# alasdairtran/transform-and-tell

Hardware: AMD Instinct MI355X
Metric: training samples/sec (img+article->caption) (higher is better)
Workload: dtype bf16; 1 GPU; BASELINE configs[2] (= per-GPU shape of configs[3]): expt/nytimes/9_transformer_objects - full faces+objects model (4 contexts: ResNet-152 image regions, RoBERTa-large article with the 25-layer weigh_bert mix, 4 faces, 64 objects), batch 32/GPU, 512-token articles, 32 caption steps; full step = frozen encoders fwd + decoder fwd/loss/bwd + BertAdam; global_batch=32, article_len=512, caption_len=33, parallelism=dp1, step_graph_replays=193, skipped_steps=0

## Files before the change

### transform-and-tell_amd/csrc/attention.hip

```cpp
#include "common.h"
#include "options.h"
#include <type_traits>

template <typename T, int D> struct ACfg {
  static constexpr int VEC = Elem<T>::VEC;
  static constexpr int PAD = sizeof(T) == 2 ? 8 : 1;
  static constexpr int DS = D + PAD;
  static constexpr int SS = 32 + PAD;
  static constexpr int DP = D < 32 ? 32 : D;
  static constexpr int DF = DP / 32;
};

typedef __attribute__((ext_vector_type(2))) float f32x2_t;
typedef __attribute__((ext_vector_type(2))) __bf16 bf16x2_t;
__device__ __forceinline__ unsigned pack_bf16x2(float lo, float hi) {
  f32x2_t f = {lo, hi};
  bf16x2_t h = __builtin_convertvector(f, bf16x2_t);
  return *reinterpret_cast<unsigned*>(&h);
}
template <typename T, int KD>
__device__ __forceinline__ f32x16 mma32(f32x16 acc, const T* a, int as, const T* b, int bs, int lane) {
  if constexpr (sizeof(T) == 2) {
#pragma unroll
    for (int ks = 0; ks < KD; ks += 16) {
// ... 678 lines not shown
            for (int r = 0; r < 16; r += 2) {
              float k0, k1;
              tell_keep2(p.seed, salt_eff, base + (f * 32 + (r & 3) + 8 * (r >> 2)), p.thr, p.inv_keep, k0, k1);
              st[f][r] = k0 != 0.f ? st[f][r] : 0.f;
              st[f][r + 1] = k1 != 0.f ? st[f][r + 1] : 0.f;
            }
        } else {
#pragma unroll
          for (int f = 0; f < 2; ++f)
#pragma unroll
            for (int r = 0; r < 16; ++r)
              st[f][r] = tell_keep(p.seed, salt_eff, base + (f * 32 + (r & 3) + 8 * (r >> 2)), p.thr, p.inv_keep) != 0.f
                             ? st[f][r] : 0.f;
        }
      }
      ls += __shfl_xor(ls, 32, 64);
      l_run = l_run * alpha + ls;
      m_run = m_new;
      if (__any(alpha != 1.f)) {
#pragma unroll
        for (int f = 0; f < 2; ++f)
#pragma unroll
          for (int r = 0; r < 16; ++r) o[f][r] *= alpha;
      }
#pragma unroll
      for (int f = 0; f < 2; ++f)
#pragma unroll
        for (int j = 0; j < 2; ++j) {
          typedef __attribute__((ext_vector_type(4))) unsigned int pk4;
          const pk4 w = {pack_bf16x2(st[f][8 * j], st[f][8 * j + 1]), pack_bf16x2(st[f][8 * j + 2], st[f][8 * j + 3]),
                         pack_bf16x2(st[f][8 * j + 4], st[f][8 * j + 5]), pack_bf16x2(st[f][8 * j + 6], st[f][8 * j + 7])};
          const bf16x8 pf = __builtin_bit_cast(bf16x8, w);
          const T* vrow = Vb + (f * 32 + j * 16) * VS;
#pragma unroll
          for (int dt = 0; dt < 2; ++dt) {
            const bf16x8 vf = attn_tr_frag(vrow + dt * 32, vrow + 8 * VS + dt * 32);
            o[dt] = __builtin_amdgcn_mfma_f32_32x32x16_bf16(vf, pf, o[dt], 0, 0, 0);
          }
        }
    }
    if (kt + 1 < nkt) RSTORE_TILE(kt + 1, buf ^ 1)
    __syncthreads();
  }
#undef RLOAD_TILE
#undef RSTORE_TILE
  if (!active || t >= p.Tq) return;
  const float inv_l = (l_run > 0.f ? 1.f / l_run : 0.f) * (DROP ? p.inv_keep : 1.f);
  T* og = static_cast<T*>(p.out) + t * p.o_st + b * p.o_sb + (long)h * D;
#pragma unroll
  for (int dt = 0; dt < 2; ++dt)
#pragma unroll
    for (int g = 0; g < 4; ++g) {
      const int d0 = dt * 32 + 8 * g + 4 * hh;
      uint2 w;
      w.x = pack_bf16x2(o[dt][4 * g] * inv_l, o[dt][4 * g + 1] * inv_l);
      w.y = pack_bf16x2(o[dt][4 * g + 2] * inv_l, o[dt][4 * g + 3] * inv_l);
      *reinterpret_cast<uint2*>(og + d0) = w;
    }
  if (lane < 32 && p.lse) p.lse[(long)bh * p.Tq + t] = l_run > 0.f ? m_run + __logf(l_run) : INFINITY;
}

#define ATTN_SELF_THR 8.0f
typedef __attribute__((address_space(3))) void* attn_lds_ptr_t;
typedef const __attribute__((address_space(1))) void* attn_glb_ptr_t;
template <bool DROP, int ABL = 0, bool DMA = false>
__global__ __launch_bounds__(256, 3) void attn_self_fwd_kernel(AttnArgs p) {
  const uint32_t salt_eff = tell_step_salt(p.salt, p.step);
  using T = uint16_t;
  constexpr int D = 64, KT = 64, NW = 4;
  constexpr int KS = DMA ? 64 : 72, VS = DMA ? 64 : 96;
  __shared__ __attribute__((aligned(16))) T Ks[2][KT * KS];
  __shared__ __attribute__((aligned(16))) T Vs[2][KT * VS];
  __shared__ __attribute__((aligned(16))) float key_bias[2][KT];
  __shared__ int tile_masked[2];
  typedef __attribute__((ext_vector_type(4))) unsigned int u32x4;
  typedef __attribute__((ext_vector_type(4))) float f32x4;
  typedef __attribute__((ext_vector_type(2))) float f32x2;

  const int tid = threadIdx.x, lane = tid & 63, wave = tid >> 6, hh = lane >> 5, qi = lane & 31;
  const int bh = blockIdx.y, b = bh / p.H, h = bh % p.H;
  const int QB = (p.Tq + 31) / 32;
  const int qb = blockIdx.x * NW + wave;
  const bool active = qb < QB;
  const int t = qb * 32 + qi;
  const int nkt = p.S / KT;
  const T* qg = static_cast<const T*>(p.q);
  const T* kb = static_cast<const T*>(p.k) + (long)b * p.k_sb + (long)h * D;
  const T* vb = static_cast<const T*>(p.v) + (long)b * p.v_sb + (long)h * D;
  const uint8_t* mrow = p.mask ? p.mask + (long)b * p.S : nullptr;

  bf16x8 qf[4];
  {
    const bool ok = active && t < p.Tq;
    const T* qp = ok ? qg + (long)t * p.q_st + (long)b * p.q_sb + (long)h * D : qg;
    const u32x4 zero4 = {0u, 0u, 0u, 0u};
#pragma unroll
    for (int ks = 0; ks < 4; ++ks) {
      u32x4 v = *reinterpret_cast<const u32x4*>(qp + (ok ? 16 * ks + 8 * hh : 0));
      if (!ok) v = zero4;
      qf[ks] = __builtin_bit_cast(bf16x8, v);
    }
  }
  unsigned koff[2], voff[2];
#pragma unroll
  for (int i = 0; i < 2; ++i) {
    const int c = tid + 256 * i;
    if constexpr (DMA) {
      const int row = 8 * (2 * wave + i) + (lane >> 3), ch = (lane & 7) ^ (row & 7);
      koff[i] = (unsigned)(row * (int)p.k_ss + ch * 8);
      voff[i] = (unsigned)(row * (int)p.v_ss + ch * 8);
    } else {
      koff[i] = (unsigned)((c >> 3) * (int)p.k_ss + (c & 7) * 8);
      voff[i] = (unsigned)((c >> 3) * (int)p.v_ss + (c & 7) * 8);
    }
  }
  const int kw0 = (tid >> 3) * KS + (tid & 7) * 8, vw0 = (tid >> 3) * VS + (tid & 7) * 8;
  u32x4 rk[2], rv[2];
  auto rload = [&](int kt) __attribute__((always_inline)) {
    const T* kt_b = kb + (long)kt * KT * p.k_ss;
    const T* vt_b = vb + (long)kt * KT * p.v_ss;
#pragma unroll
    for (int i = 0; i < 2; ++i) {
      rk[i] = *reinterpret_cast<const u32x4*>(kt_b + koff[i]);
      rv[i] = *reinterpret_cast<const u32x4*>(vt_b + voff[i]);
    }
  };
  auto dma = [&](int kt, auto buf_c) __attribute__((always_inline)) {
    constexpr int BUF = decltype(buf_c)::value;
    const T* kt_b = kb + (long)kt * KT * p.k_ss;
    const T* vt_b = vb + (long)kt * KT * p.v_ss;
#pragma unroll
    for (int i = 0; i < 2; ++i) {
      __builtin_amdgcn_global_load_lds((attn_glb_ptr_t)(kt_b + koff[i]), (attn_lds_ptr_t)&Ks[BUF][8 * (2 * wave + i) * KS], 16, 0, 0);
      __builtin_amdgcn_global_load_lds((attn_glb_ptr_t)(vt_b + voff[i]), (attn_lds_ptr_t)&Vs[BUF][8 * (2 * wave + i) * VS], 16, 0, 0);
    }
  };
  auto rstore = [&](int kt, auto buf_c) __attribute__((always_inline)) {
    constexpr int BUF = decltype(buf_c)::value;
    if constexpr (!DMA) {
#pragma unroll
      for (int i = 0; i < 2; ++i) {
        *reinterpret_cast<u32x4*>(&Ks[BUF][kw0 + i * 32 * KS]) = rk[i];
        *reinterpret_cast<u32x4*>(&Vs[BUF][vw0 + i * 32 * VS]) = rv[i];
      }
    } else {
      asm volatile("s_waitcnt vmcnt(0)" ::: "memory");
    }
    if (tid < KT) {
      const bool ok = mrow ? mrow[kt * KT + tid] == 0 : true;
      key_bias[BUF][tid] = ok ? 0.f : -INFINITY;
      const bool any_masked = __ballot(!ok) != 0;
      if (tid == 0) tile_masked[BUF] = any_masked;
    }
  };
  using B0 = std::integral_constant<int, 0>;
  using B1 = std::integral_constant<int, 1>;
  if constexpr (DMA) dma(0, B0{}); else rload(0);
  rstore(0, B0{});
  __syncthreads();

  f32x16 o[2];
#pragma unroll
  for (int f = 0; f < 2; ++f)
#pragma unroll
    for (int r = 0; r < 16; ++r) o[f][r] = 0.f;
  float m_run = -INFINITY, l_run = 0.f;
  const int k_off = qi * KS + 8 * hh;
  const int v_off = (4 * hh + ((lane & 15) >> 2)) * VS + 16 * ((lane >> 4) & 1) + 4 * (lane & 3);
  int k_sw[4], v_sw[2][2];
#pragma unroll
  for (int ks = 0; ks < 4; ++ks) k_sw[ks] = qi * 64 + (((2 * ks + hh) ^ (qi & 7)) << 3);
#pragma unroll
  for (int half = 0; half < 2; ++half)
#pragma unroll
    for (int dt = 0; dt < 2; ++dt) {
      const int r = 8 * half + 4 * hh + ((lane & 15) >> 2), c = dt * 32 + 16 * ((lane >> 4) & 1) + 4 * (lane & 3);
      v_sw[half][dt] = r * 64 + (((c >> 3) ^ (r & 7)) << 3) + (c & 7);
    }
  const uint64_t row_base = ((uint64_t)bh * p.Tq + t) * (uint64_t)p.S + 4 * hh;
  constexpr float LOG2E = 1.4426950408889634f;

  auto tile = [&](int kt, auto buf_c) __attribute__((always_inline)) {
    constexpr int BUF = decltype(buf_c)::value;
    if ((ABL & 2) == 0 && kt + 1 < nkt) {
      if constexpr (DMA) {
        if constexpr (BUF == 0) dma(kt + 1, B1{}); else dma(kt + 1, B0{});
      } else {
        rload(kt + 1);
      }
    }
    if (active) {
      const T* Kb = &Ks[BUF][k_off];
      const T* Vb = &Vs[BUF][v_off];
      f32x16 st[2];
#pragma unroll
      for (int f = 0; f < 2; ++f)
#pragma unroll
        for (int r = 0; r < 16; ++r) st[f][r] = 0.f;
#pragma unroll
      for (int ks = 0; ks < 4; ++ks)
#pragma unroll
        for (int f = 0; f < 2; ++f) {
          const bf16x8 kf = DMA ? *reinterpret_cast<const bf16x8*>(&Ks[BUF][f * 32 * 64 + k_sw[ks]])
                                : *reinterpret_cast<const bf16x8*>(Kb + f * 32 * KS + 16 * ks);
          st[f] = __builtin_amdgcn_mfma_f32_32x32x16_bf16(kf, qf[ks], st[f], 0, 0, 0);
        }
      if (__builtin_amdgcn_readfirstlane(tile_masked[BUF])) {
#pragma unroll
        for (int f = 0; f < 2; ++f)
#pragma unroll
          for (int g = 0; g < 4; ++g) {
            const f32x4 kb4 = *reinterpret_cast<const f32x4*>(&key_bias[BUF][f * 32 + 8 * g + 4 * hh]);
#pragma unroll
            for (int e = 0; e < 4; ++e) st[f][4 * g + e] += kb4[e];
          }
      }
      float mx = fmaxf(st[0][0], st[0][1]);
#pragma unroll
      for (int r = 2; r < 16; r += 2) mx = fmaxf(fmaxf(mx, st[0][r]), st[0][r + 1]);
#pragma unroll
      for (int r = 0; r < 16; r += 2) mx = fmaxf(fmaxf(mx, st[1][r]), st[1][r + 1]);
      mx = fmaxf(mx, __shfl_xor(mx, 32, 64));
      const float m_cand = fmaxf(m_run, mx);
      if (__any(!(m_cand - m_run <= ATTN_SELF_THR))) {
        const float alpha = (m_run == -INFINITY) ? 0.f : __expf(m_run - m_cand);
        m_run = m_cand;
        l_run *= alpha;
#pragma unroll
        for (int f = 0; f < 2; ++f)
#pragma unroll
          for (int r = 0; r < 16; ++r) o[f][r] *= alpha;
      }
      const float neg_m = (m_run == -INFINITY) ? 0.f : -m_run * LOG2E;
      f32x2 ls2 = {0.f, 0.f};
#pragma unroll
      for (int f = 0; f < 2; ++f)
#pragma unroll
        for (int r = 0; r < 16; r += 2) {
          const f32x2 s2 = {st[f][r], st[f][r + 1]};
          const f32x2 e2 = s2 * LOG2E + neg_m;
          const f32x2 pv = {__builtin_amdgcn_exp2f(e2[0]), __builtin_amdgcn_exp2f(e2[1])};
          ls2 += pv;
          st[f][r] = pv[0];
          st[f][r + 1] = pv[1];
        }
      float ls = ls2[0] + ls2[1];
      if constexpr (DROP) {
        const uint64_t base = row_base + (uint64_t)kt * KT;
        if (tell_keep_row_ok(base >> 2, 16)) {
          const TellKeepRow row = tell_keep_row(p.seed, salt_eff, base >> 2);
          uint32_t x = row.x0;
#pragma unroll
          for (int f = 0; f < 2; ++f)
#pragma unroll
            for (int r = 0; r < 16; r += 4) {
              bool k0, k1, k2, k3;
              tell_keep4_bits(x, row.y, p.thr, k0, k1, k2, k3);
              st[f][r] = k0 ? st[f][r] : 0.f;
              st[f][r + 1] = k1 ? st[f][r + 1] : 0.f;
              st[f][r + 2] = k2 ? st[f][r + 2] : 0.f;
              st[f][r + 3] = k3 ? st[f][r + 3] : 0.f;
              x += 2u * TELL_QUAD_STRIDE;
            }
        } else {
#pragma unroll
          for (int f = 0; f < 2; ++f)
#pragma unroll
            for (int r = 0; r < 16; r += 2) {
              float k0, k1;
              tell_keep2(p.seed, salt_eff, base + (f * 32 + (r & 3) + 8 * (r >> 2)), p.thr, p.inv_keep, k0, k1);
              st[f][r] = k0 != 0.f ? st[f][r] : 0.f;
              st[f][r + 1] = k1 != 0.f ? st[f][r + 1] : 0.f;
            }
        }
      }
      ls += __shfl_xor(ls, 32, 64);
      l_run += ls;
#pragma unroll
      for (int f = 0; f < 2; ++f)
#pragma unroll
        for (int j = 0; j < 2; ++j) {
          typedef __attribute__((ext_vector_type(4))) unsigned int pk4;
          const pk4 w = {pack_bf16x2(st[f][8 * j], st[f][8 * j + 1]), pack_bf16x2(st[f][8 * j + 2], st[f][8 * j + 3]),
                         pack_bf16x2(st[f][8 * j + 4], st[f][8 * j + 5]), pack_bf16x2(st[f][8 * j + 6], st[f][8 * j + 7])};
          const bf16x8 pf = __builtin_bit_cast(bf16x8, w);
          const T* vrow = Vb + (f * 32 + j * 16) * VS;
#pragma unroll
          for (int dt = 0; dt < 2; ++dt) {
            const T* vt = &Vs[BUF][(f * 32 + j * 16) * 64];
            const bf16x8 vf = DMA ? attn_tr_frag(vt + v_sw[0][dt], vt + v_sw[1][dt])
                                  : attn_tr_frag(vrow + dt * 32, vrow + 8 * VS + dt * 32);
            o[dt] = __builtin_amdgcn_mfma_f32_32x32x16_bf16(vf, pf, o[dt], 0, 0, 0);
          }
        }
    }
    if ((ABL & 2) == 0 && kt + 1 < nkt) {
      if constexpr (BUF == 0) rstore(kt + 1, B1{}); else rstore(kt + 1, B0{});
    }
    if ((ABL & 1) == 0) __syncthreads();
  };
  for (int kt = 0; kt < nkt; kt += 2) {
    tile(kt, B0{});
    if (kt + 1 < nkt) tile(kt + 1, B1{});
  }
  if (!active || t >= p.Tq) return;
  const float inv_l = (l_run > 0.f ? 1.f / l_run : 0.f) * (DROP ? p.inv_keep : 1.f);
  T* og = static_cast<T*>(p.out) + (long)t * p.o_st + (long)b * p.o_sb + (long)h * D;
#pragma unroll
  for (int dt = 0; dt < 2; ++dt)
#pragma unroll
    for (int g = 0; g < 4; ++g) {
      const int d0 = dt * 32 + 8 * g + 4 * hh;
      uint2 w;
      w.x = pack_bf16x2(o[dt][4 * g] * inv_l, o[dt][4 * g + 1] * inv_l);
      w.y = pack_bf16x2(o[dt][4 * g + 2] * inv_l, o[dt][4 * g + 3] * inv_l);
      *reinterpret_cast<uint2*>(og + d0) = w;
    }
  if (lane < 32 && p.lse) p.lse[(long)bh * p.Tq + t] = l_run > 0.f ? m_run + __logf(l_run) : INFINITY;
}

__device__ __forceinline__ bf16x8 attn_km_frag(const uint16_t* tile, int ld, int m0, int ks, int lane) {
  const uint16_t* p = tile + (ks + 8 * (lane >> 5) + ((lane & 15) >> 2)) * ld + m0 + 16 * ((lane >> 4) & 1) + 4 * (lane & 3);
  return attn_tr_frag(p, p + 4 * ld);
}
__device__ __forceinline__ f32x16 mma32_kmA(f32x16 acc, const uint16_t* a_km, int ald, int m0, const uint16_t* b, int bs, int lane) {
#pragma unroll
  for (int ks = 0; ks < 32; ks += 16) {
    const bf16x8 av = attn_km_frag(a_km, ald, m0, ks, lane);
    const bf16x8 bv = *reinterpret_cast<const bf16x8*>(b + (lane & 31) * bs + ks + ((lane >> 5) << 3));
    acc = __builtin_amdgcn_mfma_f32_32x32x16_bf16(av, bv, acc, 0, 0, 0);
  }
  return acc;
}
__device__ __forceinline__ f32x16 mma32_kmB(f32x16 acc, const uint16_t* a, int as, const uint16_t* b_km, int bld, int n0, int lane) {
#pragma unroll
  for (int ks = 0; ks < 32; ks += 16) {
    const bf16x8 av = *reinterpret_cast<const bf16x8*>(a + (lane & 31) * as + ks + ((lane >> 5) << 3));
    const bf16x8 bv = attn_km_frag(b_km, bld, n0, ks, lane);
    acc = __builtin_amdgcn_mfma_f32_32x32x16_bf16(av, bv, acc, 0, 0, 0);
  }
  return acc;
}

template <typename T, int D, int NW>
__global__ __launch_bounds__(64 * NW, (sizeof(T) == 2 && D == 64 && NW == 4) ? 2 : 1) void attn_bwd_kernel(AttnArgs p) {
  const uint32_t salt_eff = tell_step_salt(p.salt, p.step);
  using C_ = ACfg<T, D>;
  constexpr int DS = C_::DS, SS = C_::SS, DP = C_::DP, DF = C_::DF;
  constexpr bool TR = sizeof(T) == 2 && D == 64;
  constexpr int SHARED_ELEMS = 2 * 32 * DS + (TR ? 0 : 2 * DP * SS);
  constexpr int WAVE_ELEMS = 2 * 32 * DS + (TR ? 0 : DP * SS) + 3 * 32 * SS;
  static_assert(WAVE_ELEMS * sizeof(T) >= 16 * DF * 64 * sizeof(float), "dQ combine buffer must fit");
  __shared__ __attribute__((aligned(16))) T smem[SHARED_ELEMS + NW * WAVE_ELEMS];
  __shared__ float lse_s[32], delta_s[32];
  __shared__ float key_ok[NW][32];

  const int tid = threadIdx.x, lane = tid & 63, wave = tid >> 6;
  const int bh = blockIdx.x, b = bh / p.H, h = bh % p.H;
  const int QB = (p.Tq + 31) / 32;
  const int S_total = p.S + p.has_bias + p.has_zero;
  const int nkt = (S_total + 31) / 32;
  const int iters = (nkt + NW - 1) / NW;
  const int qi = lane & 31;

  T* Qs = smem;
  T* dOs = Qs + 32 * DS;
  T* Qt = dOs + 32 * DS;
  T* dOt = Qt + (TR ? 0 : DP * SS);
  T* Ks = smem + SHARED_ELEMS + wave * WAVE_ELEMS;
  T* Vs = Ks + 32 * DS;
  T* Kt = Vs + 32 * DS;
  T* PdT = Kt + (TR ? 0 : DP * SS);
  T* dST = PdT + 32 * SS;
  T* dSs = dST + 32 * SS;
  const T* qg = static_cast<const T*>(p.q);
  const T* kg = static_cast<const T*>(p.k);
  const T* vg = static_cast<const T*>(p.v);
  const T* og = static_cast<const T*>(p.o);
  const T* dog = static_cast<const T*>(p.dout);
  const T* bk = static_cast<const T*>(p.bias_k);
  const T* bv = static_cast<const T*>(p.bias_v);

  if (DP > D) {
    zero_lds(Qt, 2 * DP * SS, tid, 64 * NW);
    zero_lds(Kt, DP * SS, lane, 64);
  }

  for (int qb = 0; qb < QB; ++qb) {
    const int q0 = qb * 32;
    __syncthreads();
    Tile32Regs<T, D> rk, rv;
    auto fetch = [&](int kt_) __attribute__((always_inline)) {
      const int s0_ = kt_ * 32;
      load32<T, D>(rk, lane, [&](int row) -> const T* {
        int s = s0_ + row;
        if (s < p.S) return kg + s * p.k_ss + b * p.k_sb + (long)h * D;
        if (s == p.S && p.has_bias) return bk + (long)h * D;
        return nullptr;
      }, qg);
      load32<T, D>(rv, lane, [&](int row) -> const T* {
        int s = s0_ + row;
        if (s < p.S) return vg + s * p.v_ss + b * p.v_sb + (long)h * D;
        if (s == p.S && p.has_bias) return bv + (long)h * D;
        return nullptr;
      }, qg);
    };
    if (wave < nkt) fetch(wave);
    {
      constexpr int VEC = Elem<T>::VEC, CPR = D / VEC;
      static_assert((32 * CPR) % 64 == 0 && CPR <= 16 && (CPR & (CPR - 1)) == 0, "whole waves, rows inside a wave");
      for (int c = tid; c < 32 * CPR; c += 64 * NW) {
        const int row = c / CPR, ch = c % CPR, t = q0 + row;
        const bool ok = t < p.Tq;
        const long qo = ok ? t * p.q_st + b * p.q_sb + (long)h * D + ch * VEC : 0;
        const long oo = ok ? t * p.o_st + b * p.o_sb + (long)h * D + ch * VEC : 0;
        uint4 vq = *reinterpret_cast<const uint4*>(qg + qo);
        uint4 vdo = *reinterpret_cast<const uint4*>((ok ? dog : qg) + oo);
        uint4 vo = *reinterpret_cast<const uint4*>((ok ? og : qg) + oo);
        const float lse_row = p.lse[(long)bh * p.Tq + (ok ? t : 0)];
        if (!ok) vq = vdo = vo = make_uint4(0, 0, 0, 0);
        float fdo[VEC], fo[VEC];
        unpack16(vdo, fdo, (const T*)nullptr);
        unpack16(vo, fo, (const T*)nullptr);
        float part = 0.f;
#pragma unroll
        for (int k = 0; k < VEC; ++k) part += fdo[k] * fo[k];
#pragma unroll
        for (int o = CPR / 2; o > 0; o >>= 1) part += __shfl_xor(part, o, 64);
        if (ch == 0) {
          delta_s[row] = part;
          lse_s[row] = ok ? lse_row : INFINITY;
        }
        if constexpr (sizeof(T) == 2) {
          *reinterpret_cast<uint4*>(Qs + row * DS + ch * VEC) = vq;
          *reinterpret_cast<uint4*>(dOs + row * DS + ch * VEC) = vdo;
        } else {
          float* q1 = reinterpret_cast<float*>(Qs) + row * DS + ch * VEC;
          float* q2 = reinterpret_cast<float*>(dOs) + row * DS + ch * VEC;
          q1[0] = __uint_as_float(vq.x); q1[1] = __uint_as_float(vq.y); q1[2] = __uint_as_float(vq.z); q1[3] = __uint_as_float(vq.w);
          q2[0] = __uint_as_float(vdo.x); q2[1] = __uint_as_float(vdo.y); q2[2] = __uint_as_float(vdo.z); q2[3] = __uint_as_float(vdo.w);
        }
        if constexpr (!TR) {
          const T* eq = reinterpret_cast<const T*>(&vq);
          const T* ed = reinterpret_cast<const T*>(&vdo);
#pragma unroll
          for (int k = 0; k < VEC; ++k) {
            Qt[(ch * VEC + k) * SS + row] = eq[k];
            dOt[(ch * VEC + k) * SS + row] = ed[k];
          }
        }
      }
    }
    f32x16 dq[DF];
#pragma unroll
    for (int f = 0; f < DF; ++f)
#pragma unroll
      for (int r = 0; r < 16; ++r) dq[f][r] = 0.f;

    for (int it = 0; it < iters; ++it) {
      const int kt = it * NW + wave;
      const bool tv = kt < nkt;
      const int s0 = kt * 32;
      __syncthreads();
      if (tv) {
        store32<T, D>(rk, Ks, DS, TR ? (T*)nullptr : Kt, SS, lane);
        store32<T, D>(rv, Vs, DS, (T*)nullptr, 0, lane);
        if (kt + NW < nkt) fetch(kt + NW);
        if (lane < 32) {
          const int s = s0 + lane;
          bool ok = s < S_total;
          if (ok && s < p.S && p.mask) ok = p.mask[(long)b * p.S + s] == 0;
          key_ok[wave][lane] = ok ? 1.f : 0.f;
        }
      }
      __syncthreads();
      if (tv) {
        f32x16 st, dp;
#pragma unroll
        for (int r = 0; r < 16; ++r) { st[r] = 0.f; dp[r] = 0.f; }
        st = mma32<T, D>(st, Ks, DS, Qs, DS, lane);
        dp = mma32<T, D>(dp, Vs, DS, dOs, DS, lane);
        const float lse = lse_s[qi], delta = delta_s[qi];
        const int t = q0 + qi;
        float keepv[16], dsv[16];
        if (p.thr) {
          const uint64_t base = ((uint64_t)bh * p.Tq + t) * S_total + s0;
          if ((S_total & 1) == 0) {
#pragma unroll
            for (int r = 0; r < 16; r += 2)
              tell_keep2(p.seed, salt_eff, base + acc_row(r, lane), p.thr, p.inv_keep, keepv[r], keepv[r + 1]);
          } else {
#pragma unroll
            for (int r = 0; r < 16; ++r) keepv[r] = tell_keep(p.seed, salt_eff, base + acc_row(r, lane), p.thr, p.inv_keep);
          }
        } else {
#pragma unroll
          for (int r = 0; r < 16; ++r) keepv[r] = 1.f;
        }
#pragma unroll
        for (int r = 0; r < 16; ++r) {
          const int kk = acc_row(r, lane);
          const bool ok = key_ok[wave][kk] != 0.f && t < p.Tq;
          const float pv = ok ? __expf(st[r] - lse) : 0.f;
          const float keep = keepv[r];
          const float ds = pv * (dp[r] * keep - delta);
          Elem<T>::st(PdT + kk * SS + qi, pv * keep);
          Elem<T>::st(dST + kk * SS + qi, ds);
          dsv[r] = ds;
        }
#pragma unroll
        for (int g = 0; g < 4; ++g) {
          T* pd = dSs + qi * SS + 8 * g + 4 * (lane >> 5);
          if constexpr (sizeof(T) == 2) {
            uint2 w;
            w.x = pack_bf16x2(dsv[4 * g], dsv[4 * g + 1]);
            w.y = pack_bf16x2(dsv[4 * g + 2], dsv[4 * g + 3]);
            *reinterpret_cast<uint2*>(pd) = w;
          } else {
#pragma unroll
            for (int e = 0; e < 4; ++e) Elem<T>::st(pd + e, dsv[4 * g + e]);
          }
        }
      }
      __syncthreads();
      if (tv) {
#pragma unroll
        for (int f = 0; f < DF; ++f) {
          f32x16 dv, dk;
#pragma unroll
          for (int r = 0; r < 16; ++r) { dv[r] = 0.f; dk[r] = 0.f; }
          if constexpr (TR) {
            dv = mma32_kmA(dv, dOs, DS, f * 32, PdT, SS, lane);
            dk = mma32_kmA(dk, Qs, DS, f * 32, dST, SS, lane);
            dq[f] = mma32_kmB(dq[f], dSs, SS, Ks, DS, f * 32, lane);
          } else {
            dv = mma32<T, 32>(dv, dOt + f * 32 * SS, SS, PdT, SS, lane);
            dk = mma32<T, 32>(dk, Qt + f * 32 * SS, SS, dST, SS, lane);
            dq[f] = mma32<T, 32>(dq[f], dSs, SS, Kt + f * 32 * SS, SS, lane);
          }
          const int s = s0 + (lane & 31);
          const bool real = s < p.S, isb = s == p.S && p.has_bias;
          T* pk = static_cast<T*>(p.dk) + (real ? s * p.k_ss + b * p.k_sb : 0) + (long)h * D;
          T* pv_ = static_cast<T*>(p.dv) + (real ? s * p.v_ss + b * p.v_sb : 0) + (long)h * D;
          float* gk = p.dbias_k ? p.dbias_k + (long)b * p.dbias_ld + (long)h * D : nullptr;
          float* gv = p.dbias_v ? p.dbias_v + (long)b * p.dbias_ld + (long)h * D : nullptr;
#pragma unroll
          for (int g = 0; g < 4; ++g) {
            const int d0 = f * 32 + 8 * g + 4 * (lane >> 5);
            if (d0 >= D) continue;
            float vk[4], vv[4];
#pragma unroll
            for (int e = 0; e < 4; ++e) { vk[e] = dk[4 * g + e]; vv[e] = dv[4 * g + e]; }
            if (real) {
              if (qb != 0) {
#pragma unroll
                for (int e = 0; e < 4; ++e) { vk[e] += Elem<T>::ld(pk + d0 + e); vv[e] += Elem<T>::ld(pv_ + d0 + e); }
              }
              if constexpr (sizeof(T) == 2) {
                uint2 wk, wv;
                wk.x = pack_bf16x2(vk[0], vk[1]); wk.y = pack_bf16x2(vk[2], vk[3]);
                wv.x = pack_bf16x2(vv[0], vv[1]); wv.y = pack_bf16x2(vv[2], vv[3]);
                *reinterpret_cast<uint2*>(pk + d0) = wk;
                *reinterpret_cast<uint2*>(pv_ + d0) = wv;
              } else {
                *reinterpret_cast<float4*>(pk + d0) = make_float4(vk[0], vk[1], vk[2], vk[3]);
                *reinterpret_cast<float4*>(pv_ + d0) = make_float4(vv[0], vv[1], vv[2], vv[3]);
              }
            } else if (isb) {
              float4* qk = reinterpret_cast<float4*>(gk + d0);
              float4* qv = reinterpret_cast<float4*>(gv + d0);
              if (qb == 0) {
                *qk = make_float4(vk[0], vk[1], vk[2], vk[3]);
                *qv = make_float4(vv[0], vv[1], vv[2], vv[3]);
              } else {
                const float4 ok_ = *qk, ov_ = *qv;
                *qk = make_float4(ok_.x + vk[0], ok_.y + vk[1], ok_.z + vk[2], ok_.w + vk[3]);
                *qv = make_float4(ov_.x + vv[0], ov_.y + vv[1], ov_.z + vv[2], ov_.w + vv[3]);
              }
            }
          }
        }
      }
    }
    __syncthreads();
    float* comb = reinterpret_cast<float*>(smem + SHARED_ELEMS + wave * WAVE_ELEMS);
#pragma unroll
    for (int f = 0; f < DF; ++f)
#pragma unroll
      for (int r = 0; r < 16; ++r) comb[(f * 16 + r) * 64 + lane] = dq[f][r];
    __syncthreads();
    for (int item = wave; item < DF * 16; item += NW) {
      float s = 0.f;
      for (int w = 0; w < NW; ++w)
        s += reinterpret_cast<const float*>(smem + SHARED_ELEMS + w * WAVE_ELEMS)[item * 64 + lane];
      const int f = item / 16, r = item % 16;
      const int t = q0 + acc_row(r, lane), d = f * 32 + (lane & 31);
      if (t < p.Tq && d < D)
        Elem<T>::st(static_cast<T*>(p.dq) + t * p.q_st + b * p.q_sb + (long)h * D + d, s);
    }
  }
}

template <typename T>
__global__ __launch_bounds__(256) void attn_avg_weights_kernel(const T* __restrict__ q, const T* __restrict__ k,
                                                               const float* __restrict__ lse,
                                                               const uint8_t* __restrict__ mask,
                                                               const T* __restrict__ bias_k,
                                                               float* __restrict__ w, int B, int H, int Tq,
                                                               int S, int D, long q_st, long q_sb, long k_ss,
                                                               long k_sb, int has_bias, int has_zero) {
  const int t = blockIdx.x, b = blockIdx.y;
  const int S_total = S + has_bias + has_zero;
  for (int s = threadIdx.x; s < S_total; s += 256) {
    float acc = 0.f;
    const bool masked = s < S && mask && mask[(long)b * S + s];
    if (!masked) {
      for (int h = 0; h < H; ++h) {
        const T* qp = q + t * q_st + b * q_sb + (long)h * D;
        const T* kp = s < S ? k + s * k_ss + b * k_sb + (long)h * D
                            : (s == S && has_bias ? bias_k + (long)h * D : nullptr);
        float dot = 0.f;
        if (kp) for (int d = 0; d < D; ++d) dot += Elem<T>::ld(qp + d) * Elem<T>::ld(kp + d);
        acc += __expf(dot - lse[((long)b * H + h) * Tq + t]);
      }
    }
    w[((long)b * Tq + t) * S_total + s] = acc / H;
  }
}
extern "C" int tell_attn_avg_weights(const void* q, const void* k, const float* lse, const uint8_t* mask,
                                     const void* bias_k, float* w, int B, int H, int Tq, int S, int D,
                                     long q_st, long q_sb, long k_ss, long k_sb, int has_zero, int dtype,
                                     hipStream_t stream) {
  if (B * Tq <= 0) return TELL_OK;
  dim3 grid(Tq, B);
  if (dtype == TELL_BF16)
    hipLaunchKernelGGL((attn_avg_weights_kernel<uint16_t>), grid, dim3(256), 0, stream, (const uint16_t*)q, (const uint16_t*)k, lse, mask, (const uint16_t*)bias_k, w, B, H, Tq, S, D, q_st, q_sb, k_ss, k_sb, bias_k ? 1 : 0, has_zero);
  else
    hipLaunchKernelGGL((attn_avg_weights_kernel<float>), grid, dim3(256), 0, stream, (const float*)q, (const float*)k, lse, mask, (const float*)bias_k, w, B, H, Tq, S, D, q_st, q_sb, k_ss, k_sb, bias_k ? 1 : 0, has_zero);
  return tell_check_launch("attn_avg_weights");
}

static int fill_args(AttnArgs& a, const void* q, const void* k, const void* v, void* out, float* lse,
                     const uint8_t* mask, const void* bias_k, const void* bias_v, int B, int H, int Tq,
                     int S, int D, long q_st, long q_sb, long k_ss, long k_sb, long v_ss, long v_sb,
                     long o_st, long o_sb, int has_zero, float p, uint32_t seed, uint32_t salt, int dtype) {
  TELL_REQUIRE(D == 64 || D == 16, "attention: head_dim must be 64 (or 16 for the reduced-size tests)");
  TELL_REQUIRE(B > 0 && H > 0 && Tq > 0 && S >= 0, "attention: bad sizes");
  TELL_REQUIRE((bias_k == nullptr) == (bias_v == nullptr), "attention: bias_k and bias_v go together");
  TELL_REQUIRE(S + (bias_k ? 1 : 0) + has_zero > 0, "attention: no keys");
  TELL_REQUIRE(p >= 0.f && p < 1.f, "attention: dropout p must be in [0,1)");
  const int vec = dtype == TELL_BF16 ? 8 : 4;
  TELL_REQUIRE(q_st % vec == 0 && q_sb % vec == 0 && k_ss % vec == 0 && k_sb % vec == 0 &&
               v_ss % vec == 0 && v_sb % vec == 0, "attention: strides must be multiples of a 16-byte chunk");
  TELL_REQUIRE(((uintptr_t)q & 15) == 0 && ((uintptr_t)k & 15) == 0 && ((uintptr_t)v & 15) == 0,
               "attention: q/k/v must be 16-byte aligned");
  a.q = q; a.k = k; a.v = v; a.out = out; a.lse = lse; a.mask = mask; a.bias_k = bias_k; a.bias_v = bias_v;
  a.q_st = q_st; a.q_sb = q_sb; a.k_ss = k_ss; a.k_sb = k_sb; a.v_ss = v_ss; a.v_sb = v_sb;
  a.o_st = o_st; a.o_sb = o_sb; a.B = B; a.H = H; a.Tq = Tq; a.S = S;
  a.has_bias = bias_k ? 1 : 0; a.has_zero = has_zero;
  a.thr = p > 0.f ? tell_drop_threshold(p) : 0u; a.inv_keep = 1.f / (1.f - p); a.seed = seed; a.salt = salt; a.step = g_tell_rng_step;
  a.dout = nullptr; a.o = nullptr; a.dq = a.dk = a.dv = nullptr; a.dbias_k = a.dbias_v = nullptr; a.dbias_ld = 0;
  return TELL_OK;
}

extern "C" int tell_attn_fwd(const void* q, const void* k, const void* v, void* out, float* lse,
                             const uint8_t* mask, const void* bias_k, const void* bias_v, int B, int H,
                             int Tq, int S, int D, long q_st, long q_sb, long k_ss, long k_sb, long v_ss,
                             long v_sb, long o_st, long o_sb, int has_zero, float p, uint32_t seed,
                             uint32_t salt, int dtype, hipStream_t stream) {
  AttnArgs a;
  int rc = fill_args(a, q, k, v, out, lse, mask, bias_k, bias_v, B, H, Tq, S, D, q_st, q_sb, k_ss, k_sb,
                     v_ss, v_sb, o_st, o_sb, has_zero, p, seed, salt, dtype);
  if (rc) return rc;
  const int QB = (Tq + 31) / 32;
  if (D == 64 && QB >= 4) {
    dim3 grid((QB + 3) / 4, B * H);
    const int old_path = (int)tell_opt(OPT_ATTN_TILE64);
    const bool self_env = tell_opt(OPT_ATTN_SELF) != 0;
    if (dtype == TELL_BF16 && !old_path && self_env && !a.has_bias && !a.has_zero && S % 64 == 0 &&
        (long)63 * k_ss + 64 < (1L << 31) && (long)63 * v_ss + 64 < (1L << 31)) {
      const bool dma_env = tell_opt(OPT_ATTN_DMA) == 1;
      if (dma_env) {
        if (a.thr) hipLaunchKernelGGL((attn_self_fwd_kernel<true, 0, true>), grid, dim3(256), 0, stream, a);
        else hipLaunchKernelGGL((attn_self_fwd_kernel<false, 0, true>), grid, dim3(256), 0, stream, a);
      } else if (a.thr) {
        hipLaunchKernelGGL((attn_self_fwd_kernel<true>), grid, dim3(256), 0, stream, a);
      } else hipLaunchKernelGGL((attn_self_fwd_kernel<false>), grid, dim3(256), 0, stream, a);
      return tell_check_launch("attn_self_fwd");
    }
    if (dtype == TELL_BF16 && !old_path) {
      const int occ = (int)tell_opt(OPT_ATTN_OCC);
      if (occ == 3) {
        if (a.thr) hipLaunchKernelGGL((attn_fwd_reg_kernel<true, 3>), grid, dim3(256), 0, stream, a);
        else hipLaunchKernelGGL((attn_fwd_reg_kernel<false, 3>), grid, dim3(256), 0, stream, a);
      } else if (a.thr) hipLaunchKernelGGL((attn_fwd_reg_kernel<true>), grid, dim3(256), 0, stream, a);
      else hipLaunchKernelGGL((attn_fwd_reg_kernel<false>), grid, dim3(256), 0, stream, a);
      return tell_check_launch("attn_fwd_reg");
    } else if (dtype == TELL_BF16) {
      if (a.thr) hipLaunchKernelGGL((attn_fwd_tile64_kernel<uint16_t, true>), grid, dim3(256), 0, stream, a);
      else hipLaunchKernelGGL((attn_fwd_tile64_kernel<uint16_t, false>), grid, dim3(256), 0, stream, a);
    } else {
      if (a.thr) hipLaunchKernelGGL((attn_fwd_tile64_kernel<float, true>), grid, dim3(256), 0, stream, a);
      else hipLaunchKernelGGL((attn_fwd_tile64_kernel<float, false>), grid, dim3(256), 0, stream, a);
    }
    return tell_check_launch("attn_fwd_tile64");
  }
  if (dtype == TELL_BF16) {
    constexpr int NW = 4;
    dim3 grid(QB == 1 ? 1 : (QB + NW - 1) / NW, B * H);
    if (D == 64) hipLaunchKernelGGL((attn_fwd_kernel<uint16_t, 64, NW>), grid, dim3(64 * NW), 0, stream, a);
    else hipLaunchKernelGGL((attn_fwd_kernel<uint16_t, 16, NW>), grid, dim3(64 * NW), 0, stream, a);
  } else {
    constexpr int NW = 4;
    dim3 grid(QB == 1 ? 1 : (QB + NW - 1) / NW, B * H);
    if (D == 64) hipLaunchKernelGGL((attn_fwd_kernel<float, 64, NW>), grid, dim3(64 * NW), 0, stream, a);
    else hipLaunchKernelGGL((attn_fwd_kernel<float, 16, NW>), grid, dim3(64 * NW), 0, stream, a);
  }
  return tell_check_launch("attn_fwd");
}

extern "C" int tell_attn_bwd(const void* q, const void* k, const void* v, const void* out,
                             const void* dout, const float* lse, const uint8_t* mask, const void* bias_k,
                             const void* bias_v, void* dq, void* dk, void* dv, float* dbias_k,
                             float* dbias_v, int B, int H, int Tq, int S, int D, long q_st, long q_sb,
                             long k_ss, long k_sb, long v_ss, long v_sb, long o_st, long o_sb,
                             int has_zero, float p, uint32_t seed, uint32_t salt, int dtype,
                             hipStream_t stream) {
  AttnArgs a;
  int rc = fill_args(a, q, k, v, const_cast<void*>(out), const_cast<float*>(lse), mask, bias_k, bias_v, B,
                     H, Tq, S, D, q_st, q_sb, k_ss, k_sb, v_ss, v_sb, o_st, o_sb, has_zero, p, seed, salt,
                     dtype);
  if (rc) return rc;
  TELL_REQUIRE(!bias_k || (dbias_k && dbias_v), "attention bwd: dbias buffers required with bias rows");
  a.dout = dout; a.o = out; a.dq = dq; a.dk = dk; a.dv = dv; a.dbias_k = dbias_k; a.dbias_v = dbias_v;
  a.dbias_ld = (dbias_k && dbias_v == dbias_k + (long)H * D) ? 2L * H * D : (long)H * D;
  dim3 grid(B * H);
  if (dtype == TELL_BF16) {
    const int nkt = (S + (bias_k ? 1 : 0) + has_zero + 31) / 32;
    if (D == 64 && nkt <= 1) hipLaunchKernelGGL((attn_bwd_kernel<uint16_t, 64, 1>), grid, dim3(64), 0, stream, a);
    else if (D == 64 && nkt <= 4) hipLaunchKernelGGL((attn_bwd_kernel<uint16_t, 64, 2>), grid, dim3(128), 0, stream, a);
    else if (D == 64) hipLaunchKernelGGL((attn_bwd_kernel<uint16_t, 64, 4>), grid, dim3(256), 0, stream, a);
    else hipLaunchKernelGGL((attn_bwd_kernel<uint16_t, 16, 4>), grid, dim3(256), 0, stream, a);
  } else {
    if (D == 64) hipLaunchKernelGGL((attn_bwd_kernel<float, 64, 2>), grid, dim3(128), 0, stream, a);
    else hipLaunchKernelGGL((attn_bwd_kernel<float, 16, 2>), grid, dim3(128), 0, stream, a);
  }
  return tell_check_launch("attn_bwd");
}
```

### transform-and-tell_amd/csrc/options.h

```cpp
#pragma once
#include <atomic>

#define TELL_OPTION_LIST(X)                                                                                             \
                                  \
  X(OPT_GEMM_Q4, "gemm_q4", 1)                               \
  X(OPT_GEMM_Q4E, "gemm_q4e", 1)                         \
  X(OPT_Q4_PARTIAL, "q4_partial", 1)                                                 \
  X(OPT_Q4_DYNAMIC, "q4_dynamic", 0)        \
  X(OPT_Q4_VAR, "q4_var", 0)                \
  X(OPT_GEMM_PP2, "gemm_pp2", 2)                \
  X(OPT_PP2_DYNAMIC, "pp2_dynamic", 1)                                                                                  \
  X(OPT_PP2_GRID, "pp2_grid", 0)                          \
  X(OPT_GEMM_PERSIST, "gemm_persist", 0)                                                                                \
  X(OPT_GEMM_TILE, "gemm_tile", 0)          \
                                                                \
  X(OPT_GEMM_S64, "gemm_s64", 1)                                \
  X(OPT_GEMM_SMALL, "gemm_small", 1)                                                                                    \
  X(OPT_GEMM_RING, "gemm_ring", 0)               \
  X(OPT_GEMM_SPLITK, "gemm_splitk", -1)                                                                                 \
  X(OPT_GROUP_TILE, "group_tile", 0)                                                                                    \
  X(OPT_GROUP_WIDE, "group_wide", 1)                                                                                    \
  X(OPT_GROUP_SORT, "group_sort", 1)                                                                                    \
  X(OPT_CONV_TILE, "conv_tile", 0)                  \
  X(OPT_BN_FUSE, "bn_fuse", 1)                                                                                          \
  X(OPT_BN_COMBINE, "bn_combine", 0)                                                                                    \
  X(OPT_BN_WGS, "bn_wgs", 768)                                                                                          \
                                  \
  X(OPT_ATTN_TILE64, "attn_tile64", 0)                                                                                  \
  X(OPT_ATTN_SELF, "attn_self", 1)                                                                                      \
  X(OPT_ATTN_DMA, "attn_dma", 0)                                                                                        \
  X(OPT_ATTN_OCC, "attn_occ", 2)                                                                                        \
  X(OPT_DYNCONV_LDS, "dynconv_lds", 1)                                                                                  \
  X(OPT_DYNCONV_BLOCK, "dynconv_block", 1)                                                                              \
  X(OPT_LN_VAR, "ln_var", -1)                                                            \
  X(OPT_ARGMAX_REGS, "argmax_regs", 1)                                                                                  \
  X(OPT_ADAM_VAR, "adam_var", -1)                                                   \
  X(OPT_ADAM_GRID, "adam_grid", 4096)                                                                                   \
  X(OPT_SK_ROWS, "sk_rows", 0)              \
  X(OPT_SK_SPLIT, "sk_split", 0)            \
  X(OPT_SK_TALL_WAVES, "sk_tall_waves", 4)                    \
  X(OPT_SK_STAGED, "sk_staged", 1)

#define TELL_PROBE_LIST(X)                                                                                              \
  X(PROBE_Q4_ABL, "q4_abl", 0)                     \
  X(PROBE_Q4E_VAR, "q4e_var", -1)                                                      \
  X(PROBE_PP2_ABL, "pp2_abl", 0)                                                                                        \
  X(PROBE_DCB_ABL, "dcb_abl", 0)                                                                                        \
  X(PROBE_SK_STAMP_PTR, "sk_stamp_ptr", 0)        \
  X(PROBE_SK_STAMP_SLOTS, "sk_stamp_slots", 0)

enum TellOpt {
#define TELL_X(e, k, d) e,
  TELL_OPTION_LIST(TELL_X)
#ifdef TELL_PROBES
  TELL_PROBE_LIST(TELL_X)
#endif
#undef TELL_X
  TELL_OPT_COUNT
};

extern std::atomic<long> g_tell_opt[TELL_OPT_COUNT];
static inline long tell_opt(int o) { return g_tell_opt[o].load(std::memory_order_relaxed); }
#ifdef TELL_PROBES
#define tell_probe(e) tell_opt(e)
#else
#define tell_probe(e) 0L
#endif
```

Before: 1653 samples/s.

## Add attn_self2 forward kernel with padded LDS, packed dropout, and optional QK pipelining

Adds a new bf16 self-attention forward kernel, enabled by default through a new option (value 1: non-pipelined, occupancy 3). K and V tiles get separate padded LDS layouts, and a per-tile flag skips adding the key mask bias when no key in the tile is masked. Dropout is applied as saturating 16-bit masks on the packed probabilities. An optional mode computes QK for the next tile while the current tile's PV runs. The aim is to lower LDS bank conflicts and ALU work in the softmax and dropout path, at the cost of extra code paths and possible register pressure under the higher occupancy target.

Measured after the change: 1665 samples/s, median of 6. About the same (+0.7%).

```diff
diff --git a/transform-and-tell_amd/csrc/attention.hip b/transform-and-tell_amd/csrc/attention.hip
--- a/transform-and-tell_amd/csrc/attention.hip
+++ b/transform-and-tell_amd/csrc/attention.hip
@@ -1004,6 +1004,272 @@
   for (int kt = 0; kt < nkt; kt += 2) {
     tile(kt, B0{});
     if (kt + 1 < nkt) tile(kt + 1, B1{});
+  }
+  if (!active || t >= p.Tq) return;
+  const float inv_l = (l_run > 0.f ? 1.f / l_run : 0.f) * (DROP ? p.inv_keep : 1.f);
+  T* og = static_cast<T*>(p.out) + (long)t * p.o_st + (long)b * p.o_sb + (long)h * D;
+#pragma unroll
+  for (int dt = 0; dt < 2; ++dt)
+#pragma unroll
+    for (int g = 0; g < 4; ++g) {
+      const int d0 = dt * 32 + 8 * g + 4 * hh;
+      uint2 w;
+      w.x = pack_bf16x2(o[dt][4 * g] * inv_l, o[dt][4 * g + 1] * inv_l);
+      w.y = pack_bf16x2(o[dt][4 * g + 2] * inv_l, o[dt][4 * g + 3] * inv_l);
+      *reinterpret_cast<uint2*>(og + d0) = w;
+    }
+  if (lane < 32 && p.lse) p.lse[(long)bh * p.Tq + t] = l_run > 0.f ? m_run + __logf(l_run) : INFINITY;
+}
+
+template <bool DROP, bool PIPE, int OCC>
+__global__ __launch_bounds__(256, OCC) void attn_self2_fwd_kernel(AttnArgs p) {
+  const uint32_t salt_eff = tell_step_salt(p.salt, p.step);
+  using T = uint16_t;
+  constexpr int D = 64, KT = 64, NW = 4, KS = 72, VS = 96;
+  __shared__ __attribute__((aligned(16))) T Ks[2][KT * KS];
+  __shared__ __attribute__((aligned(16))) T Vs[2][KT * VS];
+  __shared__ __attribute__((aligned(16))) float key_bias[2][KT];
+  __shared__ int tile_masked[2];
+  typedef __attribute__((ext_vector_type(4))) unsigned int u32x4;
+  typedef __attribute__((ext_vector_type(4))) float f32x4;
+  typedef __attribute__((ext_vector_type(2))) float f32x2;
+  typedef __attribute__((ext_vector_type(2))) unsigned short u16x2;
+  typedef __attribute__((ext_vector_type(2))) short s16x2;
+
+  const int tid = threadIdx.x, lane = tid & 63, wave = tid >> 6, hh = lane >> 5, qi = lane & 31;
+  const int bh = blockIdx.y, b = bh / p.H, h = bh % p.H;
+  const int QB = (p.Tq + 31) / 32;
+  const int qb = blockIdx.x * NW + wave;
+  const bool active = qb < QB;
+  const int t = qb * 32 + qi;
+  const int nkt = p.S / KT;
+  const T* qg = static_cast<const T*>(p.q);
+  const T* kb = static_cast<const T*>(p.k) + (long)b * p.k_sb + (long)h * D;
+  const T* vb = static_cast<const T*>(p.v) + (long)b * p.v_sb + (long)h * D;
+  const uint8_t* mrow = p.mask ? p.mask + (long)b * p.S : nullptr;
+
+  bf16x8 qf[4];
+  {
+    const bool ok = active && t < p.Tq;
+    const T* qp = ok ? qg + (long)t * p.q_st + (long)b * p.q_sb + (long)h * D : qg;
+    const u32x4 zero4 = {0u, 0u, 0u, 0u};
+#pragma unroll
+    for (int ks = 0; ks < 4; ++ks) {
+      u32x4 v = *reinterpret_cast<const u32x4*>(qp + (ok ? 16 * ks + 8 * hh : 0));
+      if (!ok) v = zero4;
+      qf[ks] = __builtin_bit_cast(bf16x8, v);
+    }
+  }
+  unsigned koff[2], voff[2];
+#pragma unroll
+  for (int i = 0; i < 2; ++i) {
+    const int c = tid + 256 * i;
+    koff[i] = (unsigned)((c >> 3) * (int)p.k_ss + (c & 7) * 8);
+    voff[i] = (unsigned)((c >> 3) * (int)p.v_ss + (c & 7) * 8);
+  }
+  const int kw0 = (tid >> 3) * KS + (tid & 7) * 8, vw0 = (tid >> 3) * VS + (tid & 7) * 8;
+  u32x4 rk[2], rv[2];
+  auto load_k = [&](int kt) __attribute__((always_inline)) {
+    const T* kt_b = kb + (long)kt * KT * p.k_ss;
+#pragma unroll
+    for (int i = 0; i < 2; ++i) rk[i] = *reinterpret_cast<const u32x4*>(kt_b + koff[i]);
+  };
+  auto load_v = [&](int kt) __attribute__((always_inline)) {
+    const T* vt_b = vb + (long)kt * KT * p.v_ss;
+#pragma unroll
+    for (int i = 0; i < 2; ++i) rv[i] = *reinterpret_cast<const u32x4*>(vt_b + voff[i]);
+  };
+  auto store_k = [&](int kt, auto buf_c) __attribute__((always_inline)) {
+    constexpr int BUF = decltype(buf_c)::value;
+#pragma unroll
+    for (int i = 0; i < 2; ++i) *reinterpret_cast<u32x4*>(&Ks[BUF][kw0 + i * 32 * KS]) = rk[i];
+    if (tid < KT) {
+      const bool ok = mrow ? mrow[kt * KT + tid] == 0 : true;
+      key_bias[BUF][tid] = ok ? 0.f : -INFINITY;
+      const bool any_masked = __ballot(!ok) != 0;
+      if (tid == 0) tile_masked[BUF] = any_masked;
+    }
+  };
+  auto store_v = [&](auto buf_c) __attribute__((always_inline)) {
+    constexpr int BUF = decltype(buf_c)::value;
+#pragma unroll
+    for (int i = 0; i < 2; ++i) *reinterpret_cast<u32x4*>(&Vs[BUF][vw0 + i * 32 * VS]) = rv[i];
+  };
+  using B0 = std::integral_constant<int, 0>;
+  using B1 = std::integral_constant<int, 1>;
+
+  f32x16 o[2];
+#pragma unroll
+  for (int f = 0; f < 2; ++f)
+#pragma unroll
+    for (int r = 0; r < 16; ++r) o[f][r] = 0.f;
+  float m_run = -INFINITY, l_run = 0.f;
+  const int k_off = qi * KS + 8 * hh;
+  const int v_off = (4 * hh + ((lane & 15) >> 2)) * VS + 16 * ((lane >> 4) & 1) + 4 * (lane & 3);
+  const uint64_t row_base = ((uint64_t)bh * p.Tq + t) * (uint64_t)p.S + 4 * hh;
+  constexpr float LOG2E = 1.4426950408889634f;
+  const unsigned keep_add = (0x8000u - p.thr) * 0x10001u;
+
+  auto qk = [&](auto buf_c, f32x16 (&sc)[2]) __attribute__((always_inline)) {
+    constexpr int BUF = decltype(buf_c)::value;
+    const T* Kb = &Ks[BUF][k_off];
+    const f32x16 zero16 = {0.f, 0.f, 0.f, 0.f, 0.f, 0.f, 0.f, 0.f, 0.f, 0.f, 0.f, 0.f, 0.f, 0.f, 0.f, 0.f};
+#pragma unroll
+    for (int ks = 0; ks < 4; ++ks)
+#pragma unroll
+      for (int f = 0; f < 2; ++f) {
+        const bf16x8 kf = *reinterpret_cast<const bf16x8*>(Kb + f * 32 * KS + 16 * ks);
+        sc[f] = __builtin_amdgcn_mfma_f32_32x32x16_bf16(kf, qf[ks], ks == 0 ? zero16 : sc[f], 0, 0, 0);
+      }
+  };
+  auto bias_max = [&](auto buf_c, f32x16 (&sc)[2]) __attribute__((always_inline)) -> float {
+    constexpr int BUF = decltype(buf_c)::value;
+    if (__builtin_amdgcn_readfirstlane(tile_masked[BUF])) {
+#pragma unroll
+      for (int f = 0; f < 2; ++f)
+#pragma unroll
+        for (int g = 0; g < 4; ++g) {
+          const f32x4 kb4 = *reinterpret_cast<const f32x4*>(&key_bias[BUF][f * 32 + 8 * g + 4 * hh]);
+#pragma unroll
+          for (int e = 0; e < 4; ++e) sc[f][4 * g + e] += kb4[e];
+        }
+    }
+    float mx = fmaxf(sc[0][0], sc[0][1]);
+#pragma unroll
+    for (int r = 2; r < 16; r += 2) mx = fmaxf(fmaxf(mx, sc[0][r]), sc[0][r + 1]);
+#pragma unroll
+    for (int r = 0; r < 16; r += 2) mx = fmaxf(fmaxf(mx, sc[1][r]), sc[1][r + 1]);
+    const unsigned u = __float_as_uint(mx);
+    const auto sw = __builtin_amdgcn_permlane32_swap(u, u, false, false);
+    return fmaxf(__uint_as_float(sw[0]), __uint_as_float(sw[1]));
+  };
+  auto rescale = [&](float mx) __attribute__((always_inline)) {
+    const float m_cand = fmaxf(m_run, mx);
+    if (__any(!(m_cand - m_run <= ATTN_SELF_THR))) {
+      const float alpha = (m_run == -INFINITY) ? 0.f : __expf(m_run - m_cand);
+      m_run = m_cand;
+      l_run *= alpha;
+#pragma unroll
+      for (int f = 0; f < 2; ++f)
+#pragma unroll
+        for (int r = 0; r < 16; ++r) o[f][r] *= alpha;
+    }
+  };
+  auto probs_pv = [&](int kt, auto buf_c, f32x16 (&sc)[2]) __attribute__((always_inline)) {
+    constexpr int BUF = decltype(buf_c)::value;
+    const T* Vb = &Vs[BUF][v_off];
+    const float neg_m = (m_run == -INFINITY) ? 0.f : -m_run * LOG2E;
+    f32x2 ls2 = {0.f, 0.f};
+    unsigned pw[2][8];
+#pragma unroll
+    for (int f = 0; f < 2; ++f)
+#pragma unroll
+      for (int r = 0; r < 16; r += 2) {
+        const f32x2 s2 = {sc[f][r], sc[f][r + 1]};
+        const f32x2 e2 = s2 * LOG2E + neg_m;
+        const f32x2 pv = {__builtin_amdgcn_exp2f(e2[0]), __builtin_amdgcn_exp2f(e2[1])};
+        ls2 += pv;
+        pw[f][r >> 1] = pack_bf16x2(pv[0], pv[1]);
+      }
+    float ls = ls2[0] + ls2[1];
+    if constexpr (DROP) {
+      const uint64_t base = row_base + (uint64_t)kt * KT;
+      const TellKeepRow row = tell_keep_row(p.seed, salt_eff, base >> 2);
+      uint32_t x = row.x0;
+#pragma unroll
+      for (int f = 0; f < 2; ++f)
+#pragma unroll
+        for (int r = 0; r < 16; r += 4) {
+          const uint32_t hsh = tell_quad_mix(x, row.y);
+          const uint32_t ab[2] = {tell_quad_a(hsh), tell_quad_b(hsh)};
+#pragma unroll
+          for (int e = 0; e < 2; ++e) {
+            const u16x2 s = __builtin_elementwise_add_sat(__builtin_bit_cast(u16x2, ab[e]), __builtin_bit_cast(u16x2, keep_add));
+            const s16x2 m = __builtin_bit_cast(s16x2, s) >> 15;
+            pw[f][(r >> 1) + e] &= __builtin_bit_cast(unsigned, m);
+          }
+          x += 2u * TELL_QUAD_STRIDE;
+        }
+    }
+    {
+      const unsigned u = __float_as_uint(ls);
+      const auto sw = __builtin_amdgcn_permlane32_swap(u, u, false, false);
+      l_run += __uint_as_float(sw[0]) + __uint_as_float(sw[1]);
+    }
+#pragma unroll
+    for (int f = 0; f < 2; ++f)
+#pragma unroll
+      for (int j = 0; j < 2; ++j) {
+        typedef __attribute__((ext_vector_type(4))) unsigned int pk4;
+        const pk4 w = {pw[f][4 * j], pw[f][4 * j + 1], pw[f][4 * j + 2], pw[f][4 * j + 3]};
+        const bf16x8 pf = __builtin_bit_cast(bf16x8, w);
+        const T* vrow = Vb + (f * 32 + j * 16) * VS;
+#pragma unroll
+        for (int dt = 0; dt < 2; ++dt) {
+          const bf16x8 vf = attn_tr_frag(vrow + dt * 32, vrow + 8 * VS + dt * 32);
+          o[dt] = __builtin_amdgcn_mfma_f32_32x32x16_bf16(vf, pf, o[dt], 0, 0, 0);
+        }
+      }
+  };
+
+  if constexpr (!PIPE) {
+    load_k(0); load_v(0);
+    store_k(0, B0{}); store_v(B0{});
+    __syncthreads();
+    auto tile = [&](int kt, auto buf_c) __attribute__((always_inline)) {
+      constexpr int BUF = decltype(buf_c)::value;
+      using BN = std::integral_constant<int, BUF ^ 1>;
+      if (kt + 1 < nkt) { load_k(kt + 1); load_v(kt + 1); }
+      if (active) {
+        f32x16 sc[2];
+        qk(buf_c, sc);
+        rescale(bias_max(buf_c, sc));
+        probs_pv(kt, buf_c, sc);
+      }
+      if (kt + 1 < nkt) { store_k(kt + 1, BN{}); store_v(BN{}); }
+      __syncthreads();
+    };
+    for (int kt = 0; kt < nkt; kt += 2) {
+      tile(kt, B0{});
+      if (kt + 1 < nkt) tile(kt + 1, B1{});
+    }
+  } else {
+    load_k(0); load_v(0);
+    store_k(0, B0{}); store_v(B0{});
+    if (nkt > 1) { load_k(1); store_k(1, B1{}); }
+    __syncthreads();
+    f32x16 sa[2], sb[2];
+    float mx_cur = 0.f;
+    if (active) { qk(B0{}, sa); mx_cur = bias_max(B0{}, sa); }
+    auto tile = [&](int kt, auto buf_c, auto last_c, f32x16 (&cur)[2], f32x16 (&nxt)[2]) __attribute__((always_inline)) {
+      constexpr int BUF = decltype(buf_c)::value;
+      constexpr bool LAST = decltype(last_c)::value;
+      using BN = std::integral_constant<int, BUF ^ 1>;
+      if (!LAST && kt + 2 < nkt) load_k(kt + 2);
+      if (!LAST) load_v(kt + 1);
+      if (active) {
+        rescale(mx_cur);
+        if constexpr (!LAST) qk(BN{}, nxt);
+        probs_pv(kt, buf_c, cur);
+        if constexpr (!LAST) mx_cur = bias_max(BN{}, nxt);
+      }
+      if (!LAST && kt + 2 < nkt) store_k(kt + 2, buf_c);
+      if (!LAST) store_v(BN{});
+      if (!LAST) __syncthreads();
+    };
+    using F = std::false_type;
+    using L = std::true_type;
+    int kt = 0;
+    for (; kt + 2 < nkt; kt += 2) {
+      tile(kt, B0{}, F{}, sa, sb);
+      tile(kt + 1, B1{}, F{}, sb, sa);
+    }
+    if (nkt - kt == 2) {
+      tile(kt, B0{}, F{}, sa, sb);
+      tile(kt + 1, B1{}, L{}, sb, sa);
+    } else {
+      tile(kt, B0{}, L{}, sa, sb);
+    }
   }
   if (!active || t >= p.Tq) return;
   const float inv_l = (l_run > 0.f ? 1.f / l_run : 0.f) * (DROP ? p.inv_keep : 1.f);
@@ -1382,6 +1648,20 @@
     if (dtype == TELL_BF16 && !old_path && self_env && !a.has_bias && !a.has_zero && S % 64 == 0 &&
         (long)63 * k_ss + 64 < (1L << 31) && (long)63 * v_ss + 64 < (1L << 31)) {
       const bool dma_env = tell_opt(OPT_ATTN_DMA) == 1;
+      const long self2 = tell_opt(OPT_ATTN_SELF2);
+      if (self2 && !dma_env && a.thr < 0x8000u && (double)B * H * Tq * S + 64 < 17179869184.0) {
+        if (self2 == 3) {
+          if (a.thr) hipLaunchKernelGGL((attn_self2_fwd_kernel<true, true, 2>), grid, dim3(256), 0, stream, a);
+          else hipLaunchKernelGGL((attn_self2_fwd_kernel<false, true, 2>), grid, dim3(256), 0, stream, a);
+        } else if (self2 == 2) {
+          if (a.thr) hipLaunchKernelGGL((attn_self2_fwd_kernel<true, false, 2>), grid, dim3(256), 0, stream, a);
+          else hipLaunchKernelGGL((attn_self2_fwd_kernel<false, false, 2>), grid, dim3(256), 0, stream, a);
+        } else {
+          if (a.thr) hipLaunchKernelGGL((attn_self2_fwd_kernel<true, false, 3>), grid, dim3(256), 0, stream, a);
+          else hipLaunchKernelGGL((attn_self2_fwd_kernel<false, false, 3>), grid, dim3(256), 0, stream, a);
+        }
+        return tell_check_launch("attn_self2_fwd");
+      }
       if (dma_env) {
         if (a.thr) hipLaunchKernelGGL((attn_self_fwd_kernel<true, 0, true>), grid, dim3(256), 0, stream, a);
         else hipLaunchKernelGGL((attn_self_fwd_kernel<false, 0, true>), grid, dim3(256), 0, stream, a);
diff --git a/transform-and-tell_amd/csrc/options.h b/transform-and-tell_amd/csrc/options.h
--- a/transform-and-tell_amd/csrc/options.h
+++ b/transform-and-tell_amd/csrc/options.h
@@ -28,6 +28,7 @@
                                   \
   X(OPT_ATTN_TILE64, "attn_tile64", 0)                                                                                  \
   X(OPT_ATTN_SELF, "attn_self", 1)                                                                                      \
+  X(OPT_ATTN_SELF2, "attn_self2", 1)        \
   X(OPT_ATTN_DMA, "attn_dma", 0)                                                                                        \
   X(OPT_ATTN_OCC, "attn_occ", 2)                                                                                        \
   X(OPT_DYNCONV_LDS, "dynconv_lds", 1)                                                                                  \
```
